# gashon/transformer-lm

Hardware: NVIDIA B200
Metric: bpe_train_MBps (higher is better)
Workload: dtype u8

## Files before the change

transformer-lm_b200/csrc/merge.cuh:

```cuda
#pragma once
#include <cooperative_groups.h>
#include <cooperative_groups/scan.h>
#include "common.cuh"

namespace cg = cooperative_groups;

__device__ __forceinline__ u32 pair_hash(u64 key) {
    u32 h = ((u32)(key >> 32) * 0x9E3779B1u) ^ ((u32)key * 0x85EBCA77u);
    h ^= h >> 16; h *= 0x7FEB352Du; h ^= h >> 15;
    return h;
}

#define PAIR_EMPTY 0xFFFFFFFFFFFFFFFFull
#define CNT_DEAD ((i64)0x8000000000000000ll)
#define CNT_DEAD_LIMIT ((i64)0xC000000000000000ll)
#define PB 64u
#define MG_NT 512
#define MG_NEED_GROW 8ull
#ifndef MG_BATCH
#ifndef MG_BATCH
#define MG_BATCH 15u
#endif
#endif

// ... 37 lines not shown
__device__ __forceinline__ i64 sec_unpack(u32 s) { return s == SEC_SAT ? (i64)0x7FFFFFFFFFFFFFFFll : (i64)s; }

struct MergeState {
    Words W; u32 n_words;
    u64 *pkey; i64 *pcnt; u64 pcap;
    Best *bmax; u32 *bsec; uint8_t *dirty; u32 n_blocks;
    const u32 *csr_off; const Rec *csr_rec;
    Rec *log; u64 *log_rng; u64 log_cap;
    Rec *log2; u32 *bk_lg; u64 *bk_start; u32 *bk_off; u64 bk_off_cap; u32 *bk_scratch;
    u32 *tok_off; u32 *tok_len; u64 *tok_key; uint8_t *tok_bytes; u64 tok_bytes_cap;
    struct BarSlot *bar; u32 *bar_ctr;
    int stop_at;
    u32 max_batch;
    int32_t *merges_out; i64 *merge_cnt_out; int n_merges;
    int32_t *live_pairs; int live_cap;
    u64 *ctr;
    u64 *prof;
    u32 sort_min;
    u32 min_rec;
    u64 *cta_prof;
    u32 *step_prof;
};
#define MG_CTR_WORDS 64
#define MG_CTR_PENDING 16

__constant__ MergeState cM;

#ifdef BPE_MERGE_PROFILE
__device__ __forceinline__ u64 gtime_ns() { u64 t; asm volatile("mov.u64 %0, %globaltimer;" : "=l"(t)); return t; }
#define PROF_ADD(i, v) atomicAdd(&cM.prof[i], (u64)(v))
#else
__device__ __forceinline__ u64 gtime_ns() { return 0; }
#define PROF_ADD(i, v) do { } while (0)
#endif

__device__ __forceinline__ int bytes_cmp_dev(const uint8_t *x, u32 nx, const uint8_t *y, u32 ny) {
    u32 m = nx < ny ? nx : ny;
    for (u32 i = 0; i < m; i++) { if (x[i] != y[i]) return x[i] < y[i] ? -1 : 1; }
    return nx < ny ? -1 : (nx > ny ? 1 : 0);
}
__device__ __noinline__ bool tok_greater_slow(u32 p, u32 q) {
    PROF_ADD(8, 1);
    u32 lp = cM.tok_len[p], lq = cM.tok_len[q];
    if (lp <= 8 && lq <= 8) return lp > lq;
    return bytes_cmp_dev(cM.tok_bytes + cM.tok_off[p], lp, cM.tok_bytes + cM.tok_off[q], lq) > 0;
}
__device__ __forceinline__ bool best_tie_greater(u64 xkey, u64 xka, u64 xkb, u64 ykey, u64 yka, u64 ykb) {
    u32 xa = (u32)(xkey >> 32), ya = (u32)(ykey >> 32);
    if (xa != ya) return xka != yka ? xka > yka : tok_greater_slow(xa, ya);
    u32 xb = (u32)xkey, yb = (u32)ykey;
    if (xb == yb) return false;
    return xkb != ykb ? xkb > ykb : tok_greater_slow(xb, yb);
}
__device__ __noinline__ bool best_tie_greater_ni(u64 xkey, u64 xka, u64 xkb, u64 ykey, u64 yka, u64 ykb) { return best_tie_greater(xkey, xka, xkb, ykey, yka, ykb); }
// ... 59 lines not shown
    if (e.cnt < t.m2.cnt) { if (e.cnt > t.h) t.h = e.cnt; return; }
    if (best_greater(e, t.m1)) { if (t.m2.cnt > t.h) t.h = t.m2.cnt; t.m2 = t.m1; t.m1 = e; }
    else if (best_greater(e, t.m2)) { if (t.m2.cnt > t.h) t.h = t.m2.cnt; t.m2 = e; }
    else if (e.cnt > t.h) t.h = e.cnt;
}
__device__ __forceinline__ Top2 warp_top2(Top2 t) {
    Top2 r;
    r.m1 = warp_best(t.m1);
    if (r.m1.cnt != CNT_DEAD && t.m1.key == r.m1.key) { t.m1 = t.m2; t.m2 = BEST_NONE; }
    r.m2 = warp_best(t.m1);
    if (r.m2.cnt != CNT_DEAD && t.m1.key == r.m2.key) { t.m1 = t.m2; t.m2 = BEST_NONE; }
    i64 h = t.h;
    if (t.m1.cnt > h) h = t.m1.cnt;
    r.h = warp_max_cnt(h);
    return r;
}

struct __align__(16) Batch {
    u64 key[MG_BATCH]; i64 cnt[MG_BATCH];
    u64 lo[MG_BATCH], pre[MG_BATCH + 1];
    const Rec *src[MG_BATCH];
    u32 a[MG_BATCH], b[MG_BATCH], want[MG_BATCH];
    u32 r;
};
#define WANT_ANY 0xFFFFFFFFu

__device__ __forceinline__ void mark_dirty(u64 slot) { cM.dirty[(u32)(slot / PB)] = 1; }

__device__ __noinline__ void pair_add_from(u64 key, i64 delta, u64 s, u64 k) {
    const u64 mask = cM.pcap - 1;
    for (u64 probes = 0; probes < cM.pcap; probes++) {
        if (k == PAIR_EMPTY) k = atomicCAS(&cM.pkey[s], PAIR_EMPTY, key);
        if (k == PAIR_EMPTY) { atomicAdd(&cM.ctr[2], 1ull); k = key; }
        if (k == key) {
            atomicAdd((u64 *)&cM.pcnt[s], (u64)delta);
            mark_dirty(s);
            return;
        }
        s = (s + 1) & mask;
        k = cM.pkey[s];
    }
    cM.ctr[3] = 1;
}
__device__ __forceinline__ void pair_add(u32 a, u32 b, i64 delta) {
    u64 key = ((u64)a << 32) | b;
    u64 s = pair_hash(key) & (cM.pcap - 1);
    pair_add_from(key, delta, s, cM.pkey[s]);
}

__device__ __noinline__ void apply_site(u32 p, i64 c, u32 j, int step0, u32 nw0, const Batch *B) {
    int32_t *s = cM.W.sym;
    const int32_t ia = (int32_t)B->a[j], ib = (int32_t)B->b[j], inw = (int32_t)(nw0 + j);
    const int32_t tomb_hi = -(step0 + 2);
    const int32_t dead_now = tomb_hi - (int32_t)j;
#define ORIG(e) ((e) >= (int32_t)nw0 ? (int32_t)B->a[(e) - (int32_t)nw0] : ((e) <= tomb_hi ? (int32_t)B->b[tomb_hi - (e)] : (e)))
#define WAS_LIVE(e) ((e) >= 0 || (e) <= tomb_hi)
#define OLD_TOMB(e) ((e) < SYM_SEP && (e) > tomb_hi)
    int32_t vl = s[p - 1];
    const int32_t e0 = s[p];
    int32_t vb = s[p + 1], vr = s[p + 2];
    if (!WAS_LIVE(e0) || ORIG(e0) != ia) return;
    u32 pb = p + 1;
    while (OLD_TOMB(vb)) { pb++; vb = s[pb]; }
    if (!WAS_LIVE(vb) || ORIG(vb) != ib) return;
    bool has_l = false; u32 left = 0, pos_l = 0;
    u32 q = p - 1;
    while (OLD_TOMB(vl)) { q--; vl = s[q]; }
    if (ia == ib) {
        u32 n_left = 0, second = p;
        while (WAS_LIVE(vl) && ORIG(vl) == ia) {
            n_left++;
            if (n_left == 2) second = q;
            q--; vl = s[q];
            while (OLD_TOMB(vl)) { q--; vl = s[q]; }
        }
        if (n_left & 1u) return;
        if (n_left) { has_l = true; left = (u32)inw; pos_l = second; }
        else if (vl != SYM_SEP) { has_l = true; left = (u32)ORIG(vl); pos_l = q; }
    } else if (vl != SYM_SEP) {
        const int32_t o1 = ORIG(vl);
        has_l = true; left = (u32)o1; pos_l = q;
        bool looked = false; u32 q2 = q - 1; int32_t o2 = SYM_SEP;
        for (u32 i = 0; i <= j; i++) {
            if ((int32_t)B->b[i] != o1) continue;
            if (!looked) {
                int32_t v2 = s[q2];
                while (OLD_TOMB(v2)) { q2--; v2 = s[q2]; }
                o2 = WAS_LIVE(v2) ? ORIG(v2) : SYM_SEP;
                looked = true;
            }
            if (o2 == (int32_t)B->a[i]) { left = nw0 + i; pos_l = q2; break; }
        }
    }
    u32 qr = pb + 1;
    if (pb != p + 1) vr = s[qr];
    while (OLD_TOMB(vr)) { qr++; vr = s[qr]; }
    const bool has_r = vr != SYM_SEP;
    u32 right = has_r ? (u32)ORIG(vr) : 0;
    if (has_r) {
        bool looked = false; int32_t o3 = SYM_SEP;
        for (u32 i = 0; i < j; i++) {
            if (B->a[i] != right) continue;
            if (!looked) {
                u32 q3 = qr + 1;
                int32_t v3 = s[q3];
                while (OLD_TOMB(v3)) { q3++; v3 = s[q3]; }
                o3 = WAS_LIVE(v3) ? ORIG(v3) : SYM_SEP;
                looked = true;
            }
            if (o3 == (int32_t)B->b[i]) { right = nw0 + i; break; }
        }
    }
    const u32 a = (u32)ia, b = (u32)ib, nw = (u32)inw;
    const u64 mask = cM.pcap - 1;
    const u64 k0 = ((u64)left << 32) | a, k1 = ((u64)left << 32) | nw, k2 = ((u64)b << 32) | right, k3 = ((u64)nw << 32) | right;
    const u64 s0 = pair_hash(k0) & mask, s1 = pair_hash(k1) & mask, s2 = pair_hash(k2) & mask, s3 = pair_hash(k3) & mask;
    u64 v0 = 0, v1 = 0, v2 = 0, v3 = 0;
    if (has_l) { v0 = cM.pkey[s0]; v1 = atomicCAS(&cM.pkey[s1], PAIR_EMPTY, k1); }
    if (has_r) { v2 = cM.pkey[s2]; v3 = atomicCAS(&cM.pkey[s3], PAIR_EMPTY, k3); }
    const u32 n_rec = (u32)has_l + (u32)has_r;
    u64 li = 0;
    {
        const u32 act = __activemask();
        const u32 ml = __ballot_sync(act, has_l), mr = __ballot_sync(act, has_r);
        const u32 lt = (1u << lane_id()) - 1u;
        const u32 pre = __popc(ml & lt) + __popc(mr & lt), tot = __popc(ml) + __popc(mr);
        const int leader = __ffs(act) - 1;
        u64 base = 0;
        if ((int)lane_id() == leader && tot) base = atomicAdd(&cM.ctr[0], (u64)tot);
// ... 18 lines not shown
                u64 k = vv[t];
                if (k == PAIR_EMPTY) {
                    if (!((cas >> t) & 1u)) {
                        vv[t] = atomicCAS(&cM.pkey[ss[t]], PAIR_EMPTY, kk[t]);
                        cas |= 1u << t;
                        continue;
                    }
                    atomicAdd(&cM.ctr[2], 1ull);
                    k = kk[t];
                }
                if (k == kk[t]) {
                    atomicAdd((u64 *)&cM.pcnt[ss[t]], (u64)dd[t]);
                    mark_dirty(ss[t]);
                    pend &= ~(1u << t);
                    continue;
                }
                ss[t] = (ss[t] + 1) & mask;
                vv[t] = ((cas >> t) & 1u) ? atomicCAS(&cM.pkey[ss[t]], PAIR_EMPTY, kk[t]) : cM.pkey[ss[t]];
            }
        }
        if (pend) cM.ctr[3] = 1;
    }
    PROF_ADD(6, 1);
#undef ORIG
#undef WAS_LIVE
#undef OLD_TOMB
}

__device__ __noinline__ Best rescan_block(u32 blk, const u64 *prev, u32 n_prev, u32 &sec) {
    Best bst = BEST_NONE;
    i64 other = CNT_DEAD;
    const u64 sbase = (u64)blk * PB;
    u64 keys[PB / 32]; i64 cnts[PB / 32]; u64 kas[PB / 32], kbs[PB / 32];
#pragma unroll
    for (u32 k = 0; k < PB / 32; k++) { keys[k] = cM.pkey[sbase + k * 32 + lane_id()]; cnts[k] = cM.pcnt[sbase + k * 32 + lane_id()]; }
#pragma unroll
    for (u32 k = 0; k < PB / 32; k++) {
        bool live = keys[k] != PAIR_EMPTY;
        kas[k] = live ? cM.tok_key[(u32)(keys[k] >> 32)] : 0;
        kbs[k] = live ? cM.tok_key[(u32)keys[k]] : 0;
    }
#pragma unroll
    for (u32 k = 0; k < PB / 32; k++) {
        Best c;
        c.key = keys[k]; c.cnt = cnts[k]; c.ka = kas[k]; c.kb = kbs[k];
        if (c.key == PAIR_EMPTY) continue;
        bool popped = false;
        for (u32 i = 0; i < n_prev; i++) popped |= c.key == prev[i];
        if (popped) { cM.pcnt[sbase + k * 32 + lane_id()] = CNT_DEAD; continue; }
        if (c.cnt == CNT_DEAD) continue;
        if (c.cnt < CNT_DEAD_LIMIT) { c.cnt = (i64)((u64)c.cnt - (u64)CNT_DEAD); cM.pcnt[sbase + k * 32 + lane_id()] = c.cnt; }
        if (best_greater(c, bst)) { other = bst.cnt; bst = c; }
        else other = c.cnt > other ? c.cnt : other;
    }
    const Best w = warp_best(bst);
    const i64 rest = (w.cnt != CNT_DEAD && bst.key == w.key) ? other : (bst.cnt > other ? bst.cnt : other);
    sec = sec_pack(warp_max_cnt(rest));
    return w;
}

#define T_SRC(code) ((code) == 2 ? cM.csr_rec : ((code) == 1 ? (const Rec *)cM.log2 : (const Rec *)cM.log))
#define SORT_MAX_LG 12u
#define SORT_MAX_BK (1u << SORT_MAX_LG)
__device__ __forceinline__ u32 bucket_of(u32 x, u32 lg) { return (x * 0x9E3779B1u) >> (32u - lg); }

template <typename SyncFn>
__device__ __forceinline__ void sort_slice(int step0, u32 r, u64 lo, u32 n, u32 parity, bool leader_cta, u64 gthread, u64 gstride,
                                           u32 *s_scan, u32 *s_wsum, u32 *s_h, u32 *s_base, SyncFn sync) {
    u32 lg = 4;
    while ((64u << lg) < n && lg < SORT_MAX_LG) lg++;
    const u32 nbk = 1u << lg;
    const u32 tid = threadIdx.x;
    u32 *hist = cM.bk_scratch + (size_t)parity * 2 * SORT_MAX_BK;
    u32 *other = cM.bk_scratch + (size_t)(parity ^ 1u) * 2 * SORT_MAX_BK;
    for (u32 i = tid; i < nbk; i += MG_NT) s_h[i] = 0;
    __syncthreads();
    {
        u64 i = gthread;
        for (; i + 3 * gstride < n; i += 4 * gstride) {
            const u32 x0 = cM.log[lo + i].x, x1 = cM.log[lo + i + gstride].x, x2 = cM.log[lo + i + 2 * gstride].x, x3 = cM.log[lo + i + 3 * gstride].x;
            atomicAdd(&s_h[bucket_of(x0, lg)], 1u); atomicAdd(&s_h[bucket_of(x1, lg)], 1u);
// ... 72 lines not shown

struct __align__(128) BarSlot { u64 w[16]; };
#define MG_MAX_CTAS 160u
__device__ __forceinline__ u32 ld_acquire_u32(const u32 *p) { u32 v; asm volatile("ld.acquire.gpu.global.u32 %0, [%1];" : "=r"(v) : "l"(p) : "memory"); return v; }
__device__ __forceinline__ void red_release_add_u32(u32 *p, u32 v) { asm volatile("red.release.gpu.global.add.u32 [%0], %1;" ::"l"(p), "r"(v) : "memory"); }
__device__ __forceinline__ void counter_arrive_wait(u32 *counter, u32 target) {
    if (threadIdx.x == 0) {
        red_release_add_u32(counter, 1u);
        while ((int)(ld_acquire_u32(counter) - target) < 0) { }
    }
    __syncwarp();
}
__device__ __forceinline__ void grid_barrier(u32 *counter, u32 G, u32 epoch, u64 *tp = nullptr) {
    __syncthreads();
#ifdef BPE_MERGE_PROFILE
    if (tp && threadIdx.x == 0) tp[0] = gtime_ns();
#endif
    if (threadIdx.x < 32) counter_arrive_wait(counter, epoch * G);
    __syncthreads();
}

#define MG_SURV (2u * (MG_BATCH + 1u))
__device__ __noinline__ bool best_greater_ni(const Best *x, const Best *y) { return best_greater(*x, *y); }
__device__ __forceinline__ void rank_bests(const Best *s_c, const i64 *s_cnt, Best *s_surv, u32 G) {
    const u32 lane = lane_id(), warp = threadIdx.x >> 5;
    const u32 per = (G + MG_NT / 32 - 1) / (MG_NT / 32);
    i64 cj[MG_MAX_CTAS / 32];
#pragma unroll
    for (u32 m = 0; m < MG_MAX_CTAS / 32; m++) { const u32 j = lane + 32 * m; cj[m] = j < G ? s_cnt[2 * j] : CNT_DEAD; }
#pragma unroll 1
    for (u32 k = 0; k < per; k++) {
        const u32 i = warp * per + k;
        if (i >= G) break;
        const i64 ci = s_cnt[2 * i];
        if (ci == CNT_DEAD) continue;
        u32 gt = 0, eq = 0;
#pragma unroll
        for (u32 m = 0; m < MG_MAX_CTAS / 32; m++) { gt += cj[m] > ci; eq += cj[m] == ci; }
        gt = __reduce_add_sync(0xffffffffu, gt);
        eq = __reduce_add_sync(0xffffffffu, eq);
        if (gt <= MG_BATCH && eq > 1) {
            u32 extra = 0;
#pragma unroll 1
            for (u32 m = 0; m < MG_MAX_CTAS / 32; m++) {
                const u32 j = lane + 32 * m;
                if (j < G && j != i && s_cnt[2 * j] == ci && best_greater_ni(&s_c[2 * j], &s_c[2 * i])) extra++;
            }
            gt += __reduce_add_sync(0xffffffffu, extra);
        }
        if (lane == 0 && gt <= MG_BATCH) { s_surv[2 * gt] = s_c[2 * i]; s_surv[2 * gt + 1] = s_c[2 * i + 1]; }
    }
}
__device__ __noinline__ void select_batch(const Best *s_surv, Best *s_sorted, i64 H, Batch *B, u32 max_r) {
    const u32 lane = threadIdx.x;
    const Best e = lane < MG_SURV ? s_surv[lane] : BEST_NONE;
    const Best e2 = lane + 32 < MG_SURV ? s_surv[lane + 32] : BEST_NONE;
    u32 rank = 0, rank2 = 0;
#pragma unroll 1
    for (u32 m = 0; m < MG_SURV; m++) {
        const i64 cm = s_surv[m].cnt;
        if (cm > e.cnt) rank++;
        else if (cm == e.cnt && cm != CNT_DEAD && m != lane && best_greater_ni(&s_surv[m], &s_surv[lane])) rank++;
        if (MG_SURV > 32) {
            if (cm > e2.cnt) rank2++;
            else if (cm == e2.cnt && cm != CNT_DEAD && m != lane + 32 && best_greater_ni(&s_surv[m], &s_surv[lane + 32])) rank2++;
        }
    }
    if (lane <= MG_BATCH) s_sorted[lane] = BEST_NONE;
    __syncwarp();
    if (e.cnt != CNT_DEAD && rank <= MG_BATCH) s_sorted[rank] = e;
    if (MG_SURV > 32 && e2.cnt != CNT_DEAD && rank2 <= MG_BATCH) s_sorted[rank2] = e2;
    __syncwarp();
    const Best d = lane <= MG_BATCH ? s_sorted[lane] : BEST_NONE;
    const u32 a = (u32)(d.key >> 32), b = (u32)d.key;
    const u32 wT = a > b ? a : b;
    const bool have = d.cnt != CNT_DEAD, csr = wT < 256;
    u64 r_lo = 0, r_hi = 0, st0 = 0; u32 lg = 0;
    if (have) {
        if (csr) { const u32 pp = (a << 8) | b; r_lo = cM.csr_off[pp]; r_hi = cM.csr_off[pp + 1]; }
        else {
            const u32 t = wT - 256;
            const ulonglong2 rg = *reinterpret_cast<const ulonglong2 *>(&cM.log_rng[2 * (u64)t]);
            r_lo = rg.x; r_hi = rg.y; lg = cM.bk_lg[t]; st0 = cM.bk_start[t];
        }
    }
    const bool sq0 = __shfl_sync(0xffffffffu, a == b, 0);
    bool bad = !have || (lane > 0 && (a == b || sq0));
#pragma unroll 1
    for (u32 i = 0; i < MG_BATCH; i++) {
        const u32 ai = __shfl_sync(0xffffffffu, a, i), bi = __shfl_sync(0xffffffffu, b, i);
        if (i < lane) bad |= ai == b || bi == a;
    }
    const u32 first_bad = __ffs(__ballot_sync(0xffffffffu, bad || lane >= max_r)) - 1;
    const i64 next = __shfl_down_sync(0xffffffffu, d.cnt, 1);
    const bool strict = have && d.cnt > H && (next == CNT_DEAD || d.cnt > next);
    const u32 ends = __ballot_sync(0xffffffffu, lane < first_bad && strict);
    u32 good = ends ? 32u - __clz(ends) : 0u;
    const bool any = __shfl_sync(0xffffffffu, have, 0);
    if (good == 0 && any && max_r > 0) good = 1;
    u64 n = 0;
    if (lane < good) {
        const u32 want = b >= a ? a : (0x80000000u | b);
        u32 code = csr ? 2u : 0u;
        if (!csr && lg) {
            const u64 st = st0 + bucket_of(want, lg);
            const u64 base = r_lo;
            r_lo = base + cM.bk_off[st]; r_hi = base + cM.bk_off[st + 1]; code = 1u;
        }
        B->a[lane] = a; B->b[lane] = b; B->key[lane] = d.key; B->cnt[lane] = d.cnt;
        B->lo[lane] = r_lo; B->src[lane] = T_SRC(code);
        B->want[lane] = csr ? WANT_ANY : want;
        n = r_hi - r_lo;
    }
    u64 inc = n;
#pragma unroll
    for (int k = 1; k < 32; k <<= 1) { const u64 t = __shfl_up_sync(0xffffffffu, inc, k); if (lane >= (u32)k) inc += t; }
    if (lane < good) B->pre[lane + 1] = inc;
    if (lane == 0) { B->pre[0] = 0; B->r = good; }
}

__device__ __forceinline__ uint4 ldcg_v4(const void *p) { return __ldcg(reinterpret_cast<const uint4 *>(p)); }
__device__ __forceinline__ void grid_gather(BarSlot *slots, u32 *counter, u32 G, u32 epoch, const Top2 &mine, Best *s_c, i64 *s_cnt, i64 *s_h,
// ... 82 lines not shown
                const int step = step0 + (int)j;
                cM.merges_out[2 * step] = (int32_t)a; cM.merges_out[2 * step + 1] = (int32_t)b;
                cM.merge_cnt_out[step] = B->cnt[j];
                if (cM.live_pairs && step < cM.live_cap)
                    *reinterpret_cast<volatile long long *>(cM.live_pairs + 2 * step) = (long long)(((u64)b << 32) | a);
            }
            if (lane == 1) {
                const u64 key = B->key[j], mask = cM.pcap - 1;
                u64 s = pair_hash(key) & mask;
                while (cM.pkey[s] != key) s = (s + 1) & mask;
                mark_dirty(s);
            }
        }
        if (tid == 0) {
            cM.ctr[4] = cur + total;
            cM.ctr[1] = (u64)(step0 + (int)r);
            const u64 popped = cM.ctr[5];
            cM.ctr[7] += (u64)r * (live - popped) - (u64)r * (r - 1) / 2; cM.ctr[5] = popped + r;
            cM.ctr[12] += 1;
        }
    }
}

#define MG_CACHE_ITERS 4u
#define MG_CACHE_N (MG_CACHE_ITERS * (MG_NT / 32) * 64u)
#define MG_LIST_CAP 2048u
#define MG_DYN_SMEM ((size_t)MG_CACHE_N * 36 + (size_t)MG_LIST_CAP * 4 + (size_t)SORT_MAX_BK * 8)
struct BmaxCache { i64 *cnt; u64 *key, *ka, *kb; u32 *sec; };
__device__ __forceinline__ BmaxCache bmax_cache(unsigned char *base) {
    BmaxCache c;
    c.cnt = reinterpret_cast<i64 *>(base); c.key = reinterpret_cast<u64 *>(base) + MG_CACHE_N;
    c.ka = c.key + MG_CACHE_N; c.kb = c.ka + MG_CACHE_N; c.sec = reinterpret_cast<u32 *>(c.kb + MG_CACHE_N);
    return c;
}
__device__ __forceinline__ void cache_store(const BmaxCache &c, u32 i, const Best &b, u32 sec) { c.cnt[i] = b.cnt; c.key[i] = b.key; c.ka[i] = b.ka; c.kb[i] = b.kb; c.sec[i] = sec; }
__device__ __forceinline__ void cache_consider(const BmaxCache &c, u32 i, Top2 &mine) {
    const i64 s2 = sec_unpack(c.sec[i]);
    if (s2 > mine.h) mine.h = s2;
    const i64 n = c.cnt[i];
    if (n == CNT_DEAD) return;
    if (n < mine.m2.cnt) { if (n > mine.h) mine.h = n; return; }
    Best o; o.cnt = n; o.key = c.key[i]; o.ka = c.ka[i]; o.kb = c.kb[i];
    top2_add(mine, o);
}

__global__ void __launch_bounds__(MG_NT) k_merge_loop() {
    __shared__ Best s_w1[MG_NT / 32], s_w2[MG_NT / 32];
    __shared__ i64 s_wh[MG_NT / 32];
    __shared__ Best s_c[2 * MG_MAX_CTAS];
    __shared__ i64 s_cnt[2 * MG_MAX_CTAS], s_h[MG_NT / 32];
    __shared__ Best s_surv[MG_SURV + MG_BATCH + 1];
    __shared__ Batch s_B;
    __shared__ u64 s_status[2];
    __shared__ u32 s_scan[SORT_MAX_BK];
    __shared__ u32 s_wsum[32];
    __shared__ u32 s_off[MG_BATCH + 1];
    __shared__ u32 s_nd;
    extern __shared__ __align__(16) unsigned char mg_smem[];
// ... 38 lines not shown
        const bool prof_thread = false;
        u64 *ctp = nullptr;
#endif
        u64 t0 = prof_thread ? gtime_ns() : 0;
        const u32 n_prev = s_B.r;
        const u64 *prev = s_B.key;
        for (u32 it = 0; it < n_iter; it++) {
            const u32 base = (it * total_warps + gwarp) * 64;
            const u32 b0 = base + lane, b1 = base + 32 + lane;
            const bool d0 = b0 < cM.n_blocks && cM.dirty[b0], d1 = b1 < cM.n_blocks && cM.dirty[b1];
            const u32 dlo = __ballot_sync(0xffffffffu, d0), dhi = __ballot_sync(0xffffffffu, d1);
            if (dlo | dhi) {
                const u32 nlo = __popc(dlo), n = nlo + __popc(dhi);
                u32 pos = 0;
                if (lane == 0) pos = atomicAdd(&s_nd, n);
                pos = __shfl_sync(0xffffffffu, pos, 0);
                const u32 lt = (1u << lane) - 1u;
                const u32 e0 = pos + __popc(dlo & lt), e1 = pos + nlo + __popc(dhi & lt);
                if (d0 && e0 < MG_LIST_CAP) s_list[e0] = b0;
                if (d1 && e1 < MG_LIST_CAP) s_list[e1] = b1;
                if (pos + n > MG_LIST_CAP) {
                    u64 dm = (u64)__ballot_sync(0xffffffffu, d0 && e0 >= MG_LIST_CAP) | ((u64)__ballot_sync(0xffffffffu, d1 && e1 >= MG_LIST_CAP) << 32);
                    while (dm) {
                        const u32 l2 = __ffsll((long long)dm) - 1; dm &= dm - 1;
                        u32 sec;
                        const Best bst = rescan_block(base + l2, prev, n_prev, sec);
                        if (lane == 0) {
                            store_best(&cM.bmax[base + l2], bst); cM.bsec[base + l2] = sec; cM.dirty[base + l2] = 0;
                            if (it < MG_CACHE_ITERS) cache_store(sc, (it * warps_per_cta + warp) * 64 + l2, bst, sec);
                        }
                    }
                }
            }
        }
        if (tid == 0) { s_status[0] = st_err; s_status[1] = st_keys; }
        __syncthreads();
        if (s_status[0]) break;
        if (s_status[1] * 2 > cM.pcap) {
            grid_barrier(cM.bar_ctr, G, ++epoch);
            if (blockIdx.x == 0 && tid == 0) cM.ctr[3] = MG_NEED_GROW;
            break;
        }
        {
            const u32 nd = s_nd < MG_LIST_CAP ? s_nd : MG_LIST_CAP;
            for (u32 e = warp; e < nd; e += warps_per_cta) {
                const u32 blk = s_list[e];
                u32 sec;
                const Best bst = rescan_block(blk, prev, n_prev, sec);
                if (lane == 0) {
                    store_best(&cM.bmax[blk], bst); cM.bsec[blk] = sec; cM.dirty[blk] = 0; PROF_ADD(9, 1);
                    const u32 chunk = blk >> 6, it = chunk / total_warps, w = chunk - it * total_warps - blockIdx.x * warps_per_cta;
                    if (it < MG_CACHE_ITERS) cache_store(sc, (it * warps_per_cta + w) * 64 + (blk & 63u), bst, sec);
                }
            }
        }
        __syncthreads();
        if (tid == 0) s_nd = 0;
        Top2 mine = top2_none();
        for (u32 it = 0; it < n_iter; it++) {
            if (it < MG_CACHE_ITERS) {
                const u32 i0 = (it * warps_per_cta + warp) * 64 + lane;
                cache_consider(sc, i0, mine);
                cache_consider(sc, i0 + 32, mine);
            } else {
                const u32 base = (it * total_warps + gwarp) * 64;
                const u32 b0 = base + lane, b1 = base + 32 + lane;
                if (b0 < cM.n_blocks) { const i64 s2 = sec_unpack(cM.bsec[b0]); if (s2 > mine.h) mine.h = s2; top2_add(mine, load_best(&cM.bmax[b0])); }
                if (b1 < cM.n_blocks) { const i64 s2 = sec_unpack(cM.bsec[b1]); if (s2 > mine.h) mine.h = s2; top2_add(mine, load_best(&cM.bmax[b1])); }
            }
        }
        mine = warp_top2(mine);
        if (lane == 0) { s_w1[warp] = mine.m1; s_w2[warp] = mine.m2; s_wh[warp] = mine.h; }
        __syncthreads();
        Top2 cta = top2_none();
        if (warp == 0) {
            Top2 t = top2_none();
            t.m1 = lane < warps_per_cta ? s_w1[lane] : s_w2[lane - warps_per_cta];
// ... 21 lines not shown
        else {
            const u64 aw = (u64)apply_ctas * warps_per_cta;
            u32 R = 32;
            while (R > cM.min_rec && n_rec <= aw * (R >> 1)) R >>= 1;
            if (lane < R) apply_batch(step, nw0, &s_B, ((u64)warp * apply_ctas + blockIdx.x) * R + lane, aw * R);
        }
        u64 t3 = prof_thread ? gtime_ns() : 0;
        u64 tp2[2];
        grid_barrier(cM.bar_ctr, G, ++epoch, ctp ? tp2 : nullptr);
        if (ctp && tid == 0) ctp[3] = tp2[0];
        const u64 lb = *((volatile u64 *)&cM.log_rng[2 * (u64)step]), cur = *((volatile u64 *)&cM.ctr[0]);
        if (blockIdx.x == 0 && tid < r) { cM.log_rng[2 * (u64)(step + (int)tid)] = lb; cM.log_rng[2 * (u64)(step + (int)tid) + 1] = cur; }
        if (n_rec * 2 >= cM.sort_min) {
            const u64 pool = *((volatile u64 *)&cM.ctr[9]);
            if (cur - lb >= cM.sort_min && cur <= cM.log_cap && pool + SORT_MAX_BK + 1 <= cM.bk_off_cap) {
                sort_slice(step, r, lb, (u32)(cur - lb), n_sorts & 1u, blockIdx.x == 0, (u64)blockIdx.x * MG_NT + tid, (u64)G * MG_NT, s_scan, s_wsum,
                           s_sort_h, s_sort_base, [&]() { grid_barrier(cM.bar_ctr, G, ++epoch); });
                n_sorts++;
            }
        }
        if (prof_thread) {
            u64 t4 = gtime_ns();
            if (blockIdx.x == 0) {
                cM.prof[0] += t1 - t0; cM.prof[1] += t2 - t1; cM.prof[2] += t3 - t2; cM.prof[3] += t4 - t3; cM.prof[7] += 1;
                if (cM.step_prof) {
                    cM.step_prof[4 * step] = (u32)(t2 - t0); cM.step_prof[4 * step + 1] = (u32)(t4 - t2);
                    cM.step_prof[4 * step + 2] = (u32)cM.prof[5]; cM.step_prof[4 * step + 3] = r;
                }
            }
            if (token_cta) cM.prof[4] += t3 - t2;
        }
        step += (int)r;
    }
    __syncthreads();
    if (blockIdx.x == 0 && tid == 0) {
        cM.ctr[6] = s_B.r;
        for (u32 i = 0; i < s_B.r; i++) cM.ctr[MG_CTR_PENDING + i] = s_B.key[i];
    }
}

__global__ void __launch_bounds__(256) k_insert_initial_pairs(const u64 *__restrict__ dense) {
    u32 p = blockIdx.x * blockDim.x + threadIdx.x;
    if (p < 65536 && dense[p]) pair_add(p >> 8, p & 255u, (i64)dense[p]);
}

__global__ void __launch_bounds__(256) k_pairs_rehash(const u64 *__restrict__ okey, const i64 *__restrict__ ocnt, u64 ocap) {
    for (u64 i = (u64)blockIdx.x * blockDim.x + threadIdx.x; i < ocap; i += (u64)gridDim.x * blockDim.x) {
        const u64 k = okey[i];
        if (k == PAIR_EMPTY) continue;
        const i64 c = ocnt[i];
// ... 8 lines not shown
```

transformer-lm_b200/csrc/train.cu:

```cuda
#include <algorithm>
#include <cstdlib>
#include <cstring>
#include <unordered_set>
#include "kernels.h"
#include "ctx.h"
#include "merge.cuh"
#include "hashtab.cuh"
#include <cooperative_groups/reduce.h>

#define SHORT_MAX 7u
#define MED_MAX 15u
#define META_EMPTY 0ull
#define META_LEN_BITS 24
#define META_LEN_MASK ((1ull << META_LEN_BITS) - 1)
#define META_POOL_BIT (1ull << 39)
#define MAX_TOKEN_LEN ((1u << META_LEN_BITS) - 2)

struct CountTables {
    u64 *stab; u64 scap;
    u64 *mtab; u64 mcap;
    u64 *ltab; u64 lcap;
    u32 *slist, *mlist, *llist;
    ulonglong2 *hot; u64 *hcnt; u64 hot_nb;
    const uint8_t *text;
// ... 1119 lines not shown
    M.log = (Rec *)B.log.p; M.log_rng = (u64 *)B.log_rng.p; M.log_cap = log_cap;
    {
        u64 bk_cap = log_cap / 32 + (u64)(SORT_MAX_BK + 1) * 64 + 1024;
        if (const char *e = getenv("BPE_MERGE_SORTPOOL")) bk_cap = std::min<u64>(bk_cap, std::max<u64>(1, strtoull(e, nullptr, 10)));
        BPE_TRY(alloc_exact(ctx, B.log2, log_cap * sizeof(Rec))); BPE_TRY(alloc_exact(ctx, B.bk_lg, ((u64)n_merges + 2) * 4));
        BPE_TRY(alloc_exact(ctx, B.bk_start, ((u64)n_merges + 2) * 8)); BPE_TRY(alloc_exact(ctx, B.bk_off, bk_cap * 4));
        BPE_TRY(alloc_exact(ctx, B.bk_scratch, (u64)4 * SORT_MAX_BK * 4));
        CUDA_TRY(ctx, cudaMemsetAsync(B.bk_lg.p, 0, ((u64)n_merges + 2) * 4, st));
        M.log2 = (Rec *)B.log2.p; M.bk_lg = (u32 *)B.bk_lg.p; M.bk_start = (u64 *)B.bk_start.p; M.bk_off = (u32 *)B.bk_off.p;
        M.bk_off_cap = bk_cap; M.bk_scratch = (u32 *)B.bk_scratch.p;
    }
    M.tok_off = (u32 *)B.tok_off.p; M.tok_len = (u32 *)B.tok_len.p; M.tok_key = (u64 *)B.tok_key.p; M.tok_bytes = (uint8_t *)B.tok_bytes.p;
    M.tok_bytes_cap = tok_bytes_cap; M.merge_cnt_out = (i64 *)B.merge_cnt.p;
    M.live_pairs = ctx->live_pairs; M.live_cap = ctx->live_cap;
    M.merges_out = (int32_t *)B.merges.p; M.n_merges = n_merges; M.ctr = (u64 *)B.ctr.p; M.prof = (u64 *)B.prof.p;
    M.step_prof = nullptr;
    M.min_rec = 1;
    if (const char *e = getenv("BPE_MERGE_MINREC")) M.min_rec = (u32)std::max(1, std::min(32, atoi(e)));
    M.sort_min = 65536;
    if (const char *e = getenv("BPE_MERGE_SORTMIN")) M.sort_min = (u32)std::max(64, atoi(e));
    M.max_batch = MG_BATCH;
    if (const char *e = getenv("BPE_MERGE_BATCH")) M.max_batch = (u32)std::max(1, std::min((int)MG_BATCH, atoi(e)));
    if (getenv("BPE_CTA_PROFILE")) { BPE_TRY(alloc_exact(ctx, B.cta_prof, (u64)n_merges * 160 * 32)); CUDA_TRY(ctx, cudaMemsetAsync(B.cta_prof.p, 0, (u64)n_merges * 160 * 32, st)); M.cta_prof = (u64 *)B.cta_prof.p; }
    if (getenv("BPE_STEP_PROFILE")) { BPE_TRY(alloc_exact(ctx, B.step_prof, ((u64)n_merges + 1) * 16)); CUDA_TRY(ctx, cudaMemsetAsync(B.step_prof.p, 0, ((u64)n_merges + 1) * 16, st)); M.step_prof = (u32 *)B.step_prof.p; }

    CUDA_TRY(ctx, cudaMemcpyToSymbolAsync(cM, &M, sizeof(M), 0, cudaMemcpyHostToDevice, st));
    KLAUNCH(k_insert_initial_pairs, 256, 256, 0, st, (const u64 *)B.dense.p);
    CUDA_TRY(ctx, cudaGetLastError());
    int ev_build1 = tm.mark();

    {
        int per_sm = 0;
        CUDA_TRY(ctx, cudaFuncSetAttribute((void *)k_merge_loop, cudaFuncAttributeMaxDynamicSharedMemorySize, (int)MG_DYN_SMEM));
        CUDA_TRY(ctx, cudaOccupancyMaxActiveBlocksPerMultiprocessor(&per_sm, k_merge_loop, MG_NT, MG_DYN_SMEM));
        if (per_sm < 1) return bpe_set_error(ctx, BPE_ERR_CUDA, "merge kernel does not fit on an SM");
    }
    const u64 bar_bytes = (u64)MG_MAX_CTAS * sizeof(BarSlot) + 512;
    BPE_TRY(alloc_exact(ctx, B.bar, bar_bytes));
    M.bar = (BarSlot *)B.bar.p; M.bar_ctr = (u32 *)(M.bar + MG_MAX_CTAS);
    u64 ctr[MG_CTR_WORDS] = {0};
    static const bool verbose = getenv("BPE_MERGE_VERBOSE") != nullptr;
    M.stop_at = n_merges;
    for (int round = 0; n_merges > 0 && round < 64; round++) {
        CUDA_TRY(ctx, cudaMemcpyToSymbolAsync(cM, &M, sizeof(M), 0, cudaMemcpyHostToDevice, st));
        CUDA_TRY(ctx, cudaMemsetAsync(B.bk_scratch.p, 0, (u64)4 * SORT_MAX_BK * 4, st));
        CUDA_TRY(ctx, cudaMemsetAsync(B.bar.p, 0, bar_bytes, st));
        int G = std::max(2, (int)std::min<u64>((u64)std::min(ctx->sm_count, (int)MG_MAX_CTAS),
// ... 11 lines not shown
        int rc = alloc_pair_table(ocap * 4);
        if (rc != BPE_OK) { bpe_buf_free(ctx, okey); bpe_buf_free(ctx, ocnt); return rc; }
        if (verbose) fprintf(stderr, "  [pair table: %llu -> %llu slots at merge %llu, %llu keys]\n", (unsigned long long)ocap,
                             (unsigned long long)M.pcap, (unsigned long long)ctr[1], (unsigned long long)ctr[2]);
        host[3] = 0;
        CUDA_TRY(ctx, cudaMemcpyAsync((u64 *)B.ctr.p + 3, host + 3, 8, cudaMemcpyHostToDevice, st));
        ctr[3] = 0;
        unsigned rg = (unsigned)std::min<u64>((u64)ctx->sm_count * bpe_grid_mult(64), (ocap + 255) / 256);
        CUDA_TRY(ctx, cudaMemcpyToSymbolAsync(cM, &M, sizeof(M), 0, cudaMemcpyHostToDevice, st));
        KLAUNCH(k_pairs_rehash, rg, 256, 0, st, (const u64 *)okey.p, (const i64 *)ocnt.p, ocap);
        CUDA_TRY(ctx, cudaGetLastError());
        CUDA_TRY(ctx, cudaStreamSynchronize(st));
        bpe_buf_free(ctx, okey); bpe_buf_free(ctx, ocnt);
    }
    int ev_merge1 = tm.mark();
    CUDA_TRY(ctx, cudaMemcpyAsync(g_merge_prof, B.prof.p, 256, cudaMemcpyDeviceToHost, st));
    if (M.cta_prof) {
        std::vector<u64> cp((size_t)n_merges * 160 * 4);
        CUDA_TRY(ctx, cudaMemcpyAsync(cp.data(), B.cta_prof.p, cp.size() * 8, cudaMemcpyDeviceToHost, st));
        CUDA_TRY(ctx, cudaStreamSynchronize(st));
        if (FILE *f = fopen(getenv("BPE_CTA_PROFILE"), "wb")) { fwrite(cp.data(), 8, cp.size(), f); fclose(f); }
    }
    if (M.step_prof) {
        std::vector<u32> sp((size_t)n_merges * 4);
        CUDA_TRY(ctx, cudaMemcpyAsync(sp.data(), B.step_prof.p, sp.size() * 4, cudaMemcpyDeviceToHost, st));
        CUDA_TRY(ctx, cudaStreamSynchronize(st));
        if (FILE *f = fopen(getenv("BPE_STEP_PROFILE"), "wb")) { fwrite(sp.data(), 4, sp.size(), f); fclose(f); }
    }
    CUDA_TRY(ctx, cudaStreamSynchronize(st));
    if (ctr[3]) return bpe_set_error(ctx, BPE_ERR_CAPACITY, "merge loop table overflow (code %llu)", (unsigned long long)ctr[3]);
    int done = (int)ctr[1];
    if (done > 0) CUDA_TRY(ctx, cudaMemcpyAsync(merge_pairs_out, B.merges.p, (size_t)done * 8, cudaMemcpyDeviceToHost, st));
    CUDA_TRY(ctx, cudaStreamSynchronize(st));
    *n_done = done;
    u64 dup_tokens = 0;
    if (done > 0) {
        std::vector<i64> mc(done);
        CUDA_TRY(ctx, cudaMemcpyAsync(mc.data(), B.merge_cnt.p, (size_t)done * 8, cudaMemcpyDeviceToHost, st));
        CUDA_TRY(ctx, cudaStreamSynchronize(st));
        if (const char *dump = getenv("BPE_DUMP_MERGES")) {
            if (FILE *f = fopen(dump, "wb")) {
                for (int k = 0; k < done; k++) { i64 rec[3] = {merge_pairs_out[2 * k], merge_pairs_out[2 * k + 1], mc[k]}; fwrite(rec, 8, 3, f); }
                fclose(f);
            }
        }
        std::vector<std::string> sym(256);
        std::unordered_set<std::string> seen;
// ... 148 lines not shown
```

Measured before the change: 50970.

## Batch dirty-block rescans four per warp and inline tie comparisons in ranking

Replaces the per-block rescan with a routine that loads up to four dirty pair-table blocks per warp at once, so their global loads are in flight together. Each block is reduced with a cheap count-only warp max, and token keys are fetched only for the top candidates, with full tie-breaking reserved for ties. Ranking now uses an inlined tie comparator with hoisted operands instead of a noinline call. It also adds profiling counters behind compile flags. The cost is higher register pressure in the rescan and a more intricate tie-handling path.

```diff
diff --git a/transformer-lm_b200/csrc/merge.cuh b/transformer-lm_b200/csrc/merge.cuh
--- a/transformer-lm_b200/csrc/merge.cuh
+++ b/transformer-lm_b200/csrc/merge.cuh
@@ -83,6 +83,7 @@
     u32 *step_prof;
 };
 #define MG_CTR_WORDS 64
+#define MG_STEP_PROF_W 8u
 #define MG_CTR_PENDING 16
 
 __constant__ MergeState cM;
@@ -90,7 +91,9 @@
 #ifdef BPE_MERGE_PROFILE
 __device__ __forceinline__ u64 gtime_ns() { u64 t; asm volatile("mov.u64 %0, %globaltimer;" : "=l"(t)); return t; }
 #define PROF_ADD(i, v) atomicAdd(&cM.prof[i], (u64)(v))
+#define SITE_HOP (hops++)
 #else
+#define SITE_HOP ((void)0)
 __device__ __forceinline__ u64 gtime_ns() { return 0; }
 #define PROF_ADD(i, v) do { } while (0)
 #endif
@@ -196,6 +199,7 @@
     const Rec *src[MG_BATCH];
     u32 a[MG_BATCH], b[MG_BATCH], want[MG_BATCH];
     u32 r;
+    u32 capped;
 };
 #define WANT_ANY 0xFFFFFFFFu
 
@@ -230,23 +234,24 @@
 #define ORIG(e) ((e) >= (int32_t)nw0 ? (int32_t)B->a[(e) - (int32_t)nw0] : ((e) <= tomb_hi ? (int32_t)B->b[tomb_hi - (e)] : (e)))
 #define WAS_LIVE(e) ((e) >= 0 || (e) <= tomb_hi)
 #define OLD_TOMB(e) ((e) < SYM_SEP && (e) > tomb_hi)
+    u32 hops = 0; (void)hops;
     int32_t vl = s[p - 1];
     const int32_t e0 = s[p];
     int32_t vb = s[p + 1], vr = s[p + 2];
     if (!WAS_LIVE(e0) || ORIG(e0) != ia) return;
     u32 pb = p + 1;
-    while (OLD_TOMB(vb)) { pb++; vb = s[pb]; }
+    while (OLD_TOMB(vb)) { SITE_HOP; pb++; vb = s[pb]; }
     if (!WAS_LIVE(vb) || ORIG(vb) != ib) return;
     bool has_l = false; u32 left = 0, pos_l = 0;
     u32 q = p - 1;
-    while (OLD_TOMB(vl)) { q--; vl = s[q]; }
+    while (OLD_TOMB(vl)) { SITE_HOP; q--; vl = s[q]; }
     if (ia == ib) {
         u32 n_left = 0, second = p;
         while (WAS_LIVE(vl) && ORIG(vl) == ia) {
             n_left++;
             if (n_left == 2) second = q;
             q--; vl = s[q];
-            while (OLD_TOMB(vl)) { q--; vl = s[q]; }
+            while (OLD_TOMB(vl)) { SITE_HOP; q--; vl = s[q]; }
         }
         if (n_left & 1u) return;
         if (n_left) { has_l = true; left = (u32)inw; pos_l = second; }
@@ -259,7 +264,7 @@
             if ((int32_t)B->b[i] != o1) continue;
             if (!looked) {
                 int32_t v2 = s[q2];
-                while (OLD_TOMB(v2)) { q2--; v2 = s[q2]; }
+                while (OLD_TOMB(v2)) { SITE_HOP; q2--; v2 = s[q2]; }
                 o2 = WAS_LIVE(v2) ? ORIG(v2) : SYM_SEP;
                 looked = true;
             }
@@ -268,7 +273,7 @@
     }
     u32 qr = pb + 1;
     if (pb != p + 1) vr = s[qr];
-    while (OLD_TOMB(vr)) { qr++; vr = s[qr]; }
+    while (OLD_TOMB(vr)) { SITE_HOP; qr++; vr = s[qr]; }
     const bool has_r = vr != SYM_SEP;
     u32 right = has_r ? (u32)ORIG(vr) : 0;
     if (has_r) {
@@ -278,7 +283,7 @@
             if (!looked) {
                 u32 q3 = qr + 1;
                 int32_t v3 = s[q3];
-                while (OLD_TOMB(v3)) { q3++; v3 = s[q3]; }
+                while (OLD_TOMB(v3)) { SITE_HOP; q3++; v3 = s[q3]; }
                 o3 = WAS_LIVE(v3) ? ORIG(v3) : SYM_SEP;
                 looked = true;
             }
@@ -343,41 +348,105 @@
         if (pend) cM.ctr[3] = 1;
     }
     PROF_ADD(6, 1);
+    if (hops) PROF_ADD(14, hops);
 #undef ORIG
 #undef WAS_LIVE
 #undef OLD_TOMB
 }
 
-__device__ __noinline__ Best rescan_block(u32 blk, const u64 *prev, u32 n_prev, u32 &sec) {
-    Best bst = BEST_NONE;
-    i64 other = CNT_DEAD;
-    const u64 sbase = (u64)blk * PB;
-    u64 keys[PB / 32]; i64 cnts[PB / 32]; u64 kas[PB / 32], kbs[PB / 32];
-#pragma unroll
-    for (u32 k = 0; k < PB / 32; k++) { keys[k] = cM.pkey[sbase + k * 32 + lane_id()]; cnts[k] = cM.pcnt[sbase + k * 32 + lane_id()]; }
-#pragma unroll
-    for (u32 k = 0; k < PB / 32; k++) {
-        bool live = keys[k] != PAIR_EMPTY;
-        kas[k] = live ? cM.tok_key[(u32)(keys[k] >> 32)] : 0;
-        kbs[k] = live ? cM.tok_key[(u32)keys[k]] : 0;
-    }
-#pragma unroll
-    for (u32 k = 0; k < PB / 32; k++) {
-        Best c;
-        c.key = keys[k]; c.cnt = cnts[k]; c.ka = kas[k]; c.kb = kbs[k];
-        if (c.key == PAIR_EMPTY) continue;
-        bool popped = false;
-        for (u32 i = 0; i < n_prev; i++) popped |= c.key == prev[i];
-        if (popped) { cM.pcnt[sbase + k * 32 + lane_id()] = CNT_DEAD; continue; }
-        if (c.cnt == CNT_DEAD) continue;
-        if (c.cnt < CNT_DEAD_LIMIT) { c.cnt = (i64)((u64)c.cnt - (u64)CNT_DEAD); cM.pcnt[sbase + k * 32 + lane_id()] = c.cnt; }
-        if (best_greater(c, bst)) { other = bst.cnt; bst = c; }
-        else other = c.cnt > other ? c.cnt : other;
-    }
-    const Best w = warp_best(bst);
-    const i64 rest = (w.cnt != CNT_DEAD && bst.key == w.key) ? other : (bst.cnt > other ? bst.cnt : other);
-    sec = sec_pack(warp_max_cnt(rest));
-    return w;
+#define MG_CACHE_ITERS 4u
+#define MG_CACHE_N (MG_CACHE_ITERS * (MG_NT / 32) * 64u)
+#define MG_LIST_CAP 2048u
+#define MG_DYN_SMEM ((size_t)MG_CACHE_N * 36 + (size_t)MG_LIST_CAP * 4 + (size_t)SORT_MAX_BK * 8)
+struct BmaxCache { i64 *cnt; u64 *key, *ka, *kb; u32 *sec; };
+__device__ __forceinline__ BmaxCache bmax_cache(unsigned char *base) {
+    BmaxCache c;
+    c.cnt = reinterpret_cast<i64 *>(base); c.key = reinterpret_cast<u64 *>(base) + MG_CACHE_N;
+    c.ka = c.key + MG_CACHE_N; c.kb = c.ka + MG_CACHE_N; c.sec = reinterpret_cast<u32 *>(c.kb + MG_CACHE_N);
+    return c;
+}
+__device__ __forceinline__ void cache_store(const BmaxCache &c, u32 i, const Best &b, u32 sec) { c.cnt[i] = b.cnt; c.key[i] = b.key; c.ka[i] = b.ka; c.kb[i] = b.kb; c.sec[i] = sec; }
+
+#define RS_MAX 4u
+__device__ __noinline__ void rescan_blocks(u32 blk0, u32 blk1, u32 blk2, u32 blk3, u32 n, const u64 *prev, u32 n_prev,
+                                           unsigned char *smem, u32 total_warps) {
+    const u32 lane = lane_id();
+    const u32 blk[RS_MAX] = {blk0, blk1, blk2, blk3};
+    u64 keys[RS_MAX][PB / 32]; i64 cnts[RS_MAX][PB / 32];
+#pragma unroll
+    for (u32 q = 0; q < RS_MAX; q++) {
+#pragma unroll
+        for (u32 k = 0; k < PB / 32; k++) {
+            const u64 s = (u64)blk[q] * PB + k * 32 + lane;
+            keys[q][k] = PAIR_EMPTY; cnts[q][k] = CNT_DEAD;
+            if (q < n) { keys[q][k] = cM.pkey[s]; cnts[q][k] = cM.pcnt[s]; }
+        }
+    }
+    i64 m[RS_MAX], rest[RS_MAX]; u64 tk[RS_MAX]; u32 top[RS_MAX];
+#pragma unroll
+    for (u32 q = 0; q < RS_MAX; q++) {
+        m[q] = CNT_DEAD; rest[q] = CNT_DEAD; tk[q] = 0; top[q] = 0;
+        if (q >= n) continue;
+        i64 c[PB / 32];
+#pragma unroll
+        for (u32 k = 0; k < PB / 32; k++) {
+            const u64 key = keys[q][k];
+            c[k] = cnts[q][k];
+            if (key == PAIR_EMPTY) c[k] = CNT_DEAD;
+            else {
+                bool popped = false;
+                for (u32 i = 0; i < n_prev; i++) popped |= key == prev[i];
+                const u64 s = (u64)blk[q] * PB + k * 32 + lane;
+                if (popped) { cM.pcnt[s] = CNT_DEAD; c[k] = CNT_DEAD; }
+                else if (c[k] != CNT_DEAD && c[k] < CNT_DEAD_LIMIT) { c[k] = (i64)((u64)c[k] - (u64)CNT_DEAD); cM.pcnt[s] = c[k]; }
+            }
+        }
+        static_assert(PB / 32 == 2, "two slots per lane");
+        m[q] = warp_max_cnt(c[0] > c[1] ? c[0] : c[1]);
+        top[q] = m[q] == CNT_DEAD ? 0u : (c[0] == m[q] ? 1u : 0u) | (c[1] == m[q] ? 2u : 0u);
+        tk[q] = (top[q] & 1u) ? keys[q][0] : keys[q][1];
+        rest[q] = (top[q] & 1u) ? c[1] : ((top[q] & 2u) ? c[0] : (c[0] > c[1] ? c[0] : c[1]));
+    }
+    u64 ka[RS_MAX], kb[RS_MAX];
+#pragma unroll
+    for (u32 q = 0; q < RS_MAX; q++) {
+        ka[q] = top[q] ? cM.tok_key[(u32)(tk[q] >> 32)] : 0;
+        kb[q] = top[q] ? cM.tok_key[(u32)tk[q]] : 0;
+    }
+    const BmaxCache sc = bmax_cache(smem);
+#pragma unroll
+    for (u32 q = 0; q < RS_MAX; q++) {
+        if (q >= n) break;
+        Best w = BEST_NONE;
+        u32 sec = 0;
+        if (m[q] != CNT_DEAD) {
+            const u32 t1 = __ballot_sync(0xffffffffu, top[q] != 0), ntie = __popc(t1) + __popc(__ballot_sync(0xffffffffu, top[q] == 3u));
+            if (ntie == 1) {
+                const u32 src = __ffs(t1) - 1;
+                w.cnt = m[q];
+                w.key = __shfl_sync(0xffffffffu, tk[q], src);
+                w.ka = __shfl_sync(0xffffffffu, ka[q], src);
+                w.kb = __shfl_sync(0xffffffffu, kb[q], src);
+                sec = sec_pack(warp_max_cnt(rest[q]));
+            } else {
+                Best b = BEST_NONE;
+                if (top[q]) { b.cnt = m[q]; b.key = tk[q]; b.ka = ka[q]; b.kb = kb[q]; }
+                if (top[q] == 3u) {
+                    Best e; e.cnt = m[q]; e.key = keys[q][1];
+                    e.ka = cM.tok_key[(u32)(e.key >> 32)]; e.kb = cM.tok_key[(u32)e.key];
+                    if (best_greater(e, b)) b = e;
+                }
+                w = warp_best(b);
+                sec = sec_pack(m[q]);
+            }
+        }
+        if (lane == 0) {
+            const u32 bq = blk[q];
+            store_best(&cM.bmax[bq], w); cM.bsec[bq] = sec; cM.dirty[bq] = 0; PROF_ADD(9, 1);
+            const u32 chunk = bq >> 6, it = chunk / total_warps, wp = chunk - it * total_warps - blockIdx.x * (MG_NT / 32);
+            if (it < MG_CACHE_ITERS) cache_store(sc, (it * (MG_NT / 32) + wp) * 64 + (bq & 63u), w, sec);
+        }
+    }
 }
 
 #define T_SRC(code) ((code) == 2 ? cM.csr_rec : ((code) == 1 ? (const Rec *)cM.log2 : (const Rec *)cM.log))
@@ -496,6 +565,18 @@
 
 #define MG_SURV (2u * (MG_BATCH + 1u))
 __device__ __noinline__ bool best_greater_ni(const Best *x, const Best *y) { return best_greater(*x, *y); }
+__device__ __forceinline__ bool tie_greater_inl(const Best *x, u64 ykey, u64 yka, u64 ykb) {
+    const u64 xkey = x->key;
+    const u32 xa = (u32)(xkey >> 32), ya = (u32)(ykey >> 32);
+    u64 xp, yp;
+    if (xa != ya) { xp = x->ka; yp = yka; }
+    else {
+        if ((u32)xkey == (u32)ykey) return false;
+        xp = x->kb; yp = ykb;
+    }
+    if (xp != yp) return xp > yp;
+    return best_tie_greater_ni(xkey, x->ka, x->kb, ykey, yka, ykb);
+}
 __device__ __forceinline__ void rank_bests(const Best *s_c, const i64 *s_cnt, Best *s_surv, u32 G) {
     const u32 lane = lane_id(), warp = threadIdx.x >> 5;
     const u32 per = (G + MG_NT / 32 - 1) / (MG_NT / 32);
@@ -515,10 +596,11 @@
         eq = __reduce_add_sync(0xffffffffu, eq);
         if (gt <= MG_BATCH && eq > 1) {
             u32 extra = 0;
-#pragma unroll 1
+            const u64 ikey = s_c[2 * i].key, ika = s_c[2 * i].ka, ikb = s_c[2 * i].kb;
+#pragma unroll
             for (u32 m = 0; m < MG_MAX_CTAS / 32; m++) {
                 const u32 j = lane + 32 * m;
-                if (j < G && j != i && s_cnt[2 * j] == ci && best_greater_ni(&s_c[2 * j], &s_c[2 * i])) extra++;
+                if (j != i && cj[m] == ci && tie_greater_inl(&s_c[2 * j], ikey, ika, ikb)) extra++;
             }
             gt += __reduce_add_sync(0xffffffffu, extra);
         }
@@ -534,10 +616,10 @@
     for (u32 m = 0; m < MG_SURV; m++) {
         const i64 cm = s_surv[m].cnt;
         if (cm > e.cnt) rank++;
-        else if (cm == e.cnt && cm != CNT_DEAD && m != lane && best_greater_ni(&s_surv[m], &s_surv[lane])) rank++;
+        else if (cm == e.cnt && cm != CNT_DEAD && m != lane && tie_greater_inl(&s_surv[m], e.key, e.ka, e.kb)) rank++;
         if (MG_SURV > 32) {
             if (cm > e2.cnt) rank2++;
-            else if (cm == e2.cnt && cm != CNT_DEAD && m != lane + 32 && best_greater_ni(&s_surv[m], &s_surv[lane + 32])) rank2++;
+            else if (cm == e2.cnt && cm != CNT_DEAD && m != lane + 32 && tie_greater_inl(&s_surv[m], e2.key, e2.ka, e2.kb)) rank2++;
         }
     }
     if (lane <= MG_BATCH) s_sorted[lane] = BEST_NONE;
@@ -572,6 +654,13 @@
     u32 good = ends ? 32u - __clz(ends) : 0u;
     const bool any = __shfl_sync(0xffffffffu, have, 0);
     if (good == 0 && any && max_r > 0) good = 1;
+#ifdef BPE_MERGE_PROFILE
+    {
+        const u32 fb = __ffs(__ballot_sync(0xffffffffu, bad)) - 1;
+        const bool more = __shfl_sync(0xffffffffu, strict, max_r < 31 ? max_r : 31);
+        if (lane == 0) B->capped = good == max_r && fb > max_r && more;
+    }
+#endif
     u64 n = 0;
     if (lane < good) {
         const u32 want = b >= a ? a : (0x80000000u | b);
@@ -700,18 +789,6 @@
     }
 }
 
-#define MG_CACHE_ITERS 4u
-#define MG_CACHE_N (MG_CACHE_ITERS * (MG_NT / 32) * 64u)
-#define MG_LIST_CAP 2048u
-#define MG_DYN_SMEM ((size_t)MG_CACHE_N * 36 + (size_t)MG_LIST_CAP * 4 + (size_t)SORT_MAX_BK * 8)
-struct BmaxCache { i64 *cnt; u64 *key, *ka, *kb; u32 *sec; };
-__device__ __forceinline__ BmaxCache bmax_cache(unsigned char *base) {
-    BmaxCache c;
-    c.cnt = reinterpret_cast<i64 *>(base); c.key = reinterpret_cast<u64 *>(base) + MG_CACHE_N;
-    c.ka = c.key + MG_CACHE_N; c.kb = c.ka + MG_CACHE_N; c.sec = reinterpret_cast<u32 *>(c.kb + MG_CACHE_N);
-    return c;
-}
-__device__ __forceinline__ void cache_store(const BmaxCache &c, u32 i, const Best &b, u32 sec) { c.cnt[i] = b.cnt; c.key[i] = b.key; c.ka[i] = b.ka; c.kb[i] = b.kb; c.sec[i] = sec; }
 __device__ __forceinline__ void cache_consider(const BmaxCache &c, u32 i, Top2 &mine) {
     const i64 s2 = sec_unpack(c.sec[i]);
     if (s2 > mine.h) mine.h = s2;
@@ -796,13 +873,10 @@
                 if (pos + n > MG_LIST_CAP) {
                     u64 dm = (u64)__ballot_sync(0xffffffffu, d0 && e0 >= MG_LIST_CAP) | ((u64)__ballot_sync(0xffffffffu, d1 && e1 >= MG_LIST_CAP) << 32);
                     while (dm) {
-                        const u32 l2 = __ffsll((long long)dm) - 1; dm &= dm - 1;
-                        u32 sec;
-                        const Best bst = rescan_block(base + l2, prev, n_prev, sec);
-                        if (lane == 0) {
-                            store_best(&cM.bmax[base + l2], bst); cM.bsec[base + l2] = sec; cM.dirty[base + l2] = 0;
-                            if (it < MG_CACHE_ITERS) cache_store(sc, (it * warps_per_cta + warp) * 64 + l2, bst, sec);
-                        }
+                        u32 bq[RS_MAX] = {0, 0, 0, 0}, nq = 0;
+#pragma unroll
+                        for (u32 q = 0; q < RS_MAX; q++) if (dm) { bq[q] = base + __ffsll((long long)dm) - 1; dm &= dm - 1; nq++; }
+                        rescan_blocks(bq[0], bq[1], bq[2], bq[3], nq, prev, n_prev, mg_smem, total_warps);
                     }
                 }
             }
@@ -817,16 +891,15 @@
         }
         {
             const u32 nd = s_nd < MG_LIST_CAP ? s_nd : MG_LIST_CAP;
-            for (u32 e = warp; e < nd; e += warps_per_cta) {
-                const u32 blk = s_list[e];
-                u32 sec;
-                const Best bst = rescan_block(blk, prev, n_prev, sec);
-                if (lane == 0) {
-                    store_best(&cM.bmax[blk], bst); cM.bsec[blk] = sec; cM.dirty[blk] = 0; PROF_ADD(9, 1);
-                    const u32 chunk = blk >> 6, it = chunk / total_warps, w = chunk - it * total_warps - blockIdx.x * warps_per_cta;
-                    if (it < MG_CACHE_ITERS) cache_store(sc, (it * warps_per_cta + w) * 64 + (blk & 63u), bst, sec);
-                }
-            }
+            for (u32 e = warp; e < nd; e += RS_MAX * warps_per_cta) {
+                u32 bq[RS_MAX], nq = 0;
+#pragma unroll
+                for (u32 q = 0; q < RS_MAX; q++) { const u32 i = e + q * warps_per_cta; bq[q] = i < nd ? s_list[i] : 0u; nq += i < nd; }
+                rescan_blocks(bq[0], bq[1], bq[2], bq[3], nq, prev, n_prev, mg_smem, total_warps);
+            }
+#ifdef BPE_MERGE_PROFILE
+            if (tid == 0 && cM.step_prof) atomicMax(&cM.step_prof[MG_STEP_PROF_W * step + 4], (s_nd + warps_per_cta - 1) / warps_per_cta);
+#endif
         }
         __syncthreads();
         if (tid == 0) s_nd = 0;
@@ -894,10 +967,10 @@
         if (prof_thread) {
             u64 t4 = gtime_ns();
             if (blockIdx.x == 0) {
-                cM.prof[0] += t1 - t0; cM.prof[1] += t2 - t1; cM.prof[2] += t3 - t2; cM.prof[3] += t4 - t3; cM.prof[7] += 1;
+                cM.prof[0] += t1 - t0; cM.prof[1] += t2 - t1; cM.prof[2] += t3 - t2; cM.prof[3] += t4 - t3; cM.prof[7] += 1; cM.prof[15] += s_B.capped;
                 if (cM.step_prof) {
-                    cM.step_prof[4 * step] = (u32)(t2 - t0); cM.step_prof[4 * step + 1] = (u32)(t4 - t2);
-                    cM.step_prof[4 * step + 2] = (u32)cM.prof[5]; cM.step_prof[4 * step + 3] = r;
+                    u32 *sp = cM.step_prof + MG_STEP_PROF_W * step;
+                    sp[0] = (u32)(t2 - t0); sp[1] = (u32)(t4 - t2); sp[2] = (u32)cM.prof[5]; sp[3] = r; sp[5] = s_B.capped;
                 }
             }
             if (token_cta) cM.prof[4] += t3 - t2;
diff --git a/transformer-lm_b200/csrc/train.cu b/transformer-lm_b200/csrc/train.cu
--- a/transformer-lm_b200/csrc/train.cu
+++ b/transformer-lm_b200/csrc/train.cu
@@ -1165,7 +1165,7 @@
     M.max_batch = MG_BATCH;
     if (const char *e = getenv("BPE_MERGE_BATCH")) M.max_batch = (u32)std::max(1, std::min((int)MG_BATCH, atoi(e)));
     if (getenv("BPE_CTA_PROFILE")) { BPE_TRY(alloc_exact(ctx, B.cta_prof, (u64)n_merges * 160 * 32)); CUDA_TRY(ctx, cudaMemsetAsync(B.cta_prof.p, 0, (u64)n_merges * 160 * 32, st)); M.cta_prof = (u64 *)B.cta_prof.p; }
-    if (getenv("BPE_STEP_PROFILE")) { BPE_TRY(alloc_exact(ctx, B.step_prof, ((u64)n_merges + 1) * 16)); CUDA_TRY(ctx, cudaMemsetAsync(B.step_prof.p, 0, ((u64)n_merges + 1) * 16, st)); M.step_prof = (u32 *)B.step_prof.p; }
+    if (getenv("BPE_STEP_PROFILE")) { BPE_TRY(alloc_exact(ctx, B.step_prof, ((u64)n_merges + 1) * 4 * MG_STEP_PROF_W)); CUDA_TRY(ctx, cudaMemsetAsync(B.step_prof.p, 0, ((u64)n_merges + 1) * 4 * MG_STEP_PROF_W, st)); M.step_prof = (u32 *)B.step_prof.p; }
 
     CUDA_TRY(ctx, cudaMemcpyToSymbolAsync(cM, &M, sizeof(M), 0, cudaMemcpyHostToDevice, st));
     KLAUNCH(k_insert_initial_pairs, 256, 256, 0, st, (const u64 *)B.dense.p);
@@ -1223,7 +1223,7 @@
         if (FILE *f = fopen(getenv("BPE_CTA_PROFILE"), "wb")) { fwrite(cp.data(), 8, cp.size(), f); fclose(f); }
     }
     if (M.step_prof) {
-        std::vector<u32> sp((size_t)n_merges * 4);
+        std::vector<u32> sp((size_t)n_merges * MG_STEP_PROF_W);
         CUDA_TRY(ctx, cudaMemcpyAsync(sp.data(), B.step_prof.p, sp.size() * 4, cudaMemcpyDeviceToHost, st));
         CUDA_TRY(ctx, cudaStreamSynchronize(st));
         if (FILE *f = fopen(getenv("BPE_STEP_PROFILE"), "wb")) { fwrite(sp.data(), 4, sp.size(), f); fclose(f); }
```

After: 52920 (median of 6 runs). +3.8%, better.
